# tgialoimtr/cnn_lstm_ctc_ocr

Measured on AMD Instinct MI355X. Metric: line-crops/sec (train step) at 32x256 bs=256; CER vs ref, higher is better.
Workload: dtype bf16

## Files before the change

cnn_lstm_ctc_ocr_amd/csrc/gemm_w4.hip:

```cpp
#include "gemm.h"
#include "mfma_util.h"

namespace ocrk {

namespace {

constexpr unsigned W4_OOB = 0x80000000u;

__device__ __forceinline__ void w4_barrier() {
    __builtin_amdgcn_sched_barrier(0);
    asm volatile("" ::: "memory");
    __builtin_amdgcn_s_barrier();
    asm volatile("" ::: "memory");
    __builtin_amdgcn_sched_barrier(0);
}

template <int NR, int NM, int REST>
__device__ __forceinline__ void w4_interleave() {
#pragma unroll
    for (int r = 0; r < NR; ++r) {
        __builtin_amdgcn_sched_group_barrier(0x8, NM, 0);
        __builtin_amdgcn_sched_group_barrier(0x100, 1, 0);
    }
    __builtin_amdgcn_sched_group_barrier(0x8, REST, 0);
}

typedef unsigned short u16x4 __attribute__((ext_vector_type(4)));

__device__ __forceinline__ i32x4_t w4_rsrc(const void* base, int bytes) {
    const uint64_t b = (uint64_t)base;
    return i32x4_t{(int)(unsigned)b, (int)((unsigned)(b >> 32) & 0xffffu), bytes, 0x00020000};
}

__device__ __forceinline__ void w4_dma16(const i32x4_t& r, unsigned lds, unsigned voff, unsigned soff) {
    asm volatile("s_nop 0\n\tbuffer_load_dwordx4 %0, %1, %2 offen lds"
                 :: "v"(voff), "s"(r), "s"(soff), "{m0}"(lds) : "memory");
}

__global__ void __launch_bounds__(256) gemm_w4_kernel(const GemmParams p) {
    constexpr int BM = 256, BN = 256, BK = 64, ROWB = 128;
    constexpr int A_BYTES = BM * ROWB, BUF = (BM + BN) * ROWB;
    constexpr int NU = 8;
    constexpr int BIAS_OFF = 2 * BUF, STG_OFF = BIAS_OFF + 4 * 1024;
    constexpr int PITCH = 128 * 2 + 16, STG = 16 * PITCH;
    constexpr int NST = 8 * 4;
    extern __shared__ __attribute__((aligned(16))) char smem[];

    const int tid = threadIdx.x, lane = tid & 63;
    const int wave = __builtin_amdgcn_readfirstlane(tid >> 6);
    const int wm = wave >> 1, wn = wave & 1;
    const int i16 = lane & 15, g = lane >> 4, sw = lane & 7;

    const int tm = (p.M + BM - 1) / BM, tn = (p.N + BN - 1) / BN;
    const int nitems = tm * tn * p.batch;
    const int per = (nitems + 7) >> 3;
    const int xcd = blockIdx.x & 7, slot = blockIdx.x >> 3, sp = gridDim.x >> 3;
    const int wend = min(nitems, (xcd + 1) * per);
    int w_issue = xcd * per + slot;
    if (w_issue >= wend) return;

    typedef const __attribute__((address_space(4))) GemmParams* KArgs;
    const bool has_bias = p.bias != nullptr;
    const int c_nk = max(1, (p.K + BK - 1) / BK);

    const int lrow = lane >> 3;
    const int cs = (lane & 7) ^ lrow;
    i32x4_t ra, rb;
    int i_m0 = 0, i_n0 = 0, i_zb = 0, i_kt = 0, i_cnt = 0;
    const unsigned a_lane = (unsigned)(lrow * p.lda * 2), b_lane = (unsigned)(lrow * p.ldb * 2);
    auto setup_issue = [&](int w) {
        const PPItem it = pp_item(w, tm, tn, 1, BM, BN);
        ra = w4_rsrc(reinterpret_cast<const bf16*>(p.A) + it.zb * p.strideA, p.M * (int)p.lda * 2);
        rb = w4_rsrc(reinterpret_cast<const bf16*>(p.B) + it.zb * p.strideB, p.N * (int)p.ldb * 2);
        i_m0 = it.m0;
        i_n0 = it.n0;
        i_zb = it.zb;
        i_kt = 0;
    };
    int ops = 0;
    const unsigned lds0 = (unsigned)(uintptr_t)(__attribute__((address_space(3))) char*)smem;
    auto lane_off = [&](unsigned lane_row, bool on) -> unsigned {
        const int k = i_kt * BK + 8 * cs;
        return on && k < p.K ? lane_row + (unsigned)(k * 2) : W4_OOB;
    };
    auto unit_base = [&](int first, unsigned buf, int& row, unsigned& lds) {
        row = first + wave * 8;
        lds = buf + wave * 8 * ROWB;
        asm volatile("" : "+s"(row), "+s"(lds));
    };
    auto dma_a = [&](int i, int row, unsigned lds, unsigned va) {
        const int mrow = row + i * 32;
        const unsigned soff = mrow < p.M ? (unsigned)(mrow * (int)p.lda * 2) : 0u;
        w4_dma16(ra, lds + i * 32 * ROWB, lrow < p.M - mrow ? va : W4_OOB, soff);
    };
    auto dma_b = [&](int i, int row, unsigned lds, unsigned vb) {
        const int ncol = row + i * 32;
        const unsigned soff = ncol < p.N ? (unsigned)(ncol * (int)p.ldb * 2) : 0u;
        w4_dma16(rb, lds + i * 32 * ROWB, lrow < p.N - ncol ? vb : W4_OOB, soff);
    };
    auto dma_bias = [&](bool on) {
        if (i_kt == 0 && has_bias && wave == 0) {
            const int n = i_n0 + 4 * lane;
            KArgs e = (KArgs)__builtin_amdgcn_kernarg_segment_ptr();
            asm volatile("" : "+s"(e));
            const i32x4_t rbias = w4_rsrc(e->bias + i_zb * e->strideBias, p.N * 4);
            w4_dma16(rbias, lds0 + BIAS_OFF + (i_cnt & 3) * 1024, on && n < p.N ? (unsigned)(n * 4) : W4_OOB, 0u);
            ops += 1;
        }
    };
    auto advance_issue = [&]() -> bool {
        if (++i_kt < c_nk) return true;
        w_issue += sp;
        ++i_cnt;
        if (w_issue >= wend) return false;
        setup_issue(w_issue);
        return true;
    };

    int w_comp = w_issue, c_cnt = 0;

    bf16x8 af0[8], bf0[8], af1[8], bf1[8];
    const int a_base = (wm * 128 + i16) * ROWB, b_base = A_BYTES + (wn * 128 + i16) * ROWB;
    auto read_a = [&](const char* buf, int kk, bf16x8 (&fr)[8]) {
#pragma unroll
        for (int i = 0; i < 8; ++i)
            fr[i] = *reinterpret_cast<const bf16x8*>(buf + a_base + i * 16 * ROWB + (((kk * 4 + g) ^ sw) << 4));
    };
    auto read_b = [&](const char* buf, int kk, bf16x8 (&fr)[8]) {
#pragma unroll
        for (int j = 0; j < 8; ++j)
            fr[j] = *reinterpret_cast<const bf16x8*>(buf + b_base + j * 16 * ROWB + (((kk * 4 + g) ^ sw) << 4));
    };
    floatx4 acc[8][8];
    auto zero_acc = [&]() {
#pragma unroll
        for (int i = 0; i < 8; ++i)
#pragma unroll
            for (int j = 0; j < 8; ++j) acc[i][j] = floatx4{0.f, 0.f, 0.f, 0.f};
    };
    auto mfma_rows = [&](auto I0_, const bf16x8 (&a)[8], const bf16x8 (&b)[8]) {
        constexpr int I0 = decltype(I0_)::value;
#pragma unroll
        for (int i = I0; i < I0 + 4; ++i)
#pragma unroll
            for (int j = 0; j < 8; ++j)
                acc[i][j] = __builtin_amdgcn_mfma_f32_16x16x32_bf16(b[j], a[i], acc[i][j], 0, 0, 0);
    };
    using R0 = std::integral_constant<int, 0>;
    using R4 = std::integral_constant<int, 4>;
    (void)read_b;

    int mA1 = 0, mB1 = 0, mA2 = 0, mB2 = 0;
    setup_issue(w_issue);
    bool more = true;
    int m0done = 0;
#pragma unroll
    for (int t = 0; t < 2; ++t) {
        const unsigned va = lane_off(a_lane, more), vb = lane_off(b_lane, more);
        int row;
        unsigned lds;
        unit_base(i_m0, lds0 + t * BUF, row, lds);
#pragma unroll
        for (int i = 0; i < NU; ++i) dma_a(i, row, lds, va);
        ops += NU;
        mA1 = ops;
        dma_bias(more);
        unit_base(i_n0, lds0 + t * BUF + A_BYTES, row, lds);
#pragma unroll
        for (int i = 0; i < NU; ++i) dma_b(i, row, lds, vb);
        ops += NU;
        mB1 = ops;
        if (t == 0) m0done = ops;
        if (more) more = advance_issue();
    }
    vm_wait_n(ops - m0done);
    w4_barrier();
    read_a(smem, 0, af0);
    read_b(smem, 0, bf0);

    int s = 0;
    for (;;) {
      zero_acc();
      for (int c_kt = 0; c_kt < c_nk; ++c_kt) {
        char* cur = smem + (s & 1) * BUF;
        const char* nxt = smem + ((s + 1) & 1) * BUF;
        __builtin_amdgcn_sched_barrier(0);
        __builtin_amdgcn_s_setprio(1);
        read_a(cur, 1, af1);
        read_b(cur, 1, bf1);
        mfma_rows(R0{}, af0, bf0);
        mfma_rows(R4{}, af0, bf0);
        w4_interleave<16, 3, 16>();
        __builtin_amdgcn_s_setprio(0);
        __builtin_amdgcn_sched_barrier(0);
        asm volatile("s_waitcnt lgkmcnt(0)" ::: "memory");
        vm_wait_fast<NU>(ops - mA1);
        w4_barrier();
        {
            const unsigned va = lane_off(a_lane, more);
            int row;
            unsigned lds;
            unit_base(i_m0, lds0 + (s & 1) * BUF, row, lds);
            __builtin_amdgcn_s_setprio(1);
#pragma unroll
            for (int q = 0; q < 8; ++q) {
                af0[q] = *reinterpret_cast<const bf16x8*>(nxt + a_base + q * 16 * ROWB + ((g ^ sw) << 4));
#pragma unroll
                for (int j = (q & 1) * 4; j < (q & 1) * 4 + 4; ++j)
                    acc[q >> 1][j] = __builtin_amdgcn_mfma_f32_16x16x32_bf16(bf1[j], af1[q >> 1], acc[q >> 1][j], 0, 0, 0);
                dma_a(q, row, lds, va);
                __builtin_amdgcn_sched_barrier(0);
            }
            __builtin_amdgcn_s_setprio(0);
            ops += NU;
            mA2 = ops;
        }
        vm_wait_fast<NU>(ops - mB1);
        w4_barrier();
        {
            const unsigned vb = lane_off(b_lane, more);
            dma_bias(more);
            int row;
            unsigned lds;
            unit_base(i_n0, lds0 + (s & 1) * BUF + A_BYTES, row, lds);
            __builtin_amdgcn_s_setprio(1);
#pragma unroll
            for (int q = 0; q < 8; ++q) {
                bf0[q] = *reinterpret_cast<const bf16x8*>(nxt + b_base + q * 16 * ROWB + ((g ^ sw) << 4));
#pragma unroll
                for (int j = (q & 1) * 4; j < (q & 1) * 4 + 4; ++j)
                    acc[4 + (q >> 1)][j] =
                        __builtin_amdgcn_mfma_f32_16x16x32_bf16(bf1[j], af1[4 + (q >> 1)], acc[4 + (q >> 1)][j], 0, 0, 0);
                dma_b(q, row, lds, vb);
                __builtin_amdgcn_sched_barrier(0);
            }
            __builtin_amdgcn_s_setprio(0);
            ops += NU;
            mB2 = ops;
        }
        if (more) more = advance_issue();
        mA1 = mA2;
        mB1 = mB2;
        ++s;
      }

        {
            int el;
            asm volatile("v_mbcnt_lo_u32_b32 %0, -1, 0\n\tv_mbcnt_hi_u32_b32 %0, -1, %0" : "=v"(el));
            const PPItem cur_it = pp_item(w_comp, tm, tn, 1, BM, BN);
            KArgs e = (KArgs)__builtin_amdgcn_kernarg_segment_ptr();
            asm volatile("" : "+s"(e));
            const int i16 = el & 15, g = el >> 4;
            const char* bslot = smem + BIAS_OFF + (c_cnt & 3) * 1024 + (wn * 128 + 4 * g) * 4;
            floatx4 bv[8];
#pragma unroll
            for (int j = 0; j < 8; ++j) {
                bv[j] = floatx4{0.f, 0.f, 0.f, 0.f};
                if (has_bias) bv[j] = *reinterpret_cast<const floatx4*>(bslot + j * 64);
            }
            char* stg = smem + STG_OFF + wave * STG;
            bf16* Cb = reinterpret_cast<bf16*>(e->C) + cur_it.zb * e->strideC;
            const __amdgpu_buffer_rsrc_t rc =
                __builtin_amdgcn_make_buffer_rsrc(Cb, 0, ((p.M - 1) * (int)e->ldc + p.N) * 2, 0x00020000);
            const int c8 = el & 15, r0 = el >> 4;
            const int n = cur_it.n0 + wn * 128 + 8 * c8;
#pragma unroll
            for (int h = 0; h < 8; ++h) {
#pragma unroll
                for (int j = 0; j < 8; ++j) {
                    floatx4 v = acc[h][j] * e->alpha + bv[j];
                    if (e->relu) {
#pragma unroll
                        for (int r = 0; r < 4; ++r) v[r] = fmaxf(v[r], 0.f);
                    }
                    u16x4 o;
#pragma unroll
                    for (int r = 0; r < 4; ++r) o[r] = __builtin_bit_cast(unsigned short, (bf16)v[r]);
                    *reinterpret_cast<u16x4*>(stg + i16 * PITCH + (j * 16 + 4 * g) * 2) = o;
                }
                __builtin_amdgcn_wave_barrier();
#pragma unroll
                for (int q = 0; q < 4; ++q) {
                    const int r = r0 + q * 4;
                    const int m = cur_it.m0 + wm * 128 + h * 16 + r;
                    const u32x4 v = *reinterpret_cast<const u32x4*>(stg + r * PITCH + c8 * 16);
                    const unsigned off = (m < p.M && n < p.N) ? (unsigned)(((int64_t)m * e->ldc + n) * 2) : W4_OOB;
                    __builtin_amdgcn_raw_buffer_store_b128(v, rc, off, 0, 0);
                }
                __builtin_amdgcn_wave_barrier();
            }
            ops += NST;
        }
        w_comp += sp;
        ++c_cnt;
        if (w_comp >= wend) break;
    }
    vm_wait<0>();
}

}

int gemm_w4(const GemmParams& p, int amode, int bmode, int dtype, hipStream_t stream) {
    const int64_t mode = opt(OPT_GEMM_W4);
    if (mode == 0 || dtype != OCRK_BF16 || amode != A_ROWK || bmode != B_NK) return -1;
    if (!p.c_bf16 || p.accumulate || p.splits != 1 || p.mask || p.stats || p.mask_bits || p.relu_bits) return -1;
    if (p.N % 8 != 0 || p.K % 8 != 0 || (int64_t)p.M < 4096 || p.N < 96) return -1;
    if ((int64_t)p.M * p.lda * 2 >= (1ll << 31) || (int64_t)p.N * p.ldb * 2 >= (1ll << 31) ||
        (int64_t)p.M * p.ldc * 2 >= (1ll << 31))
        return -1;
    if (p.ldc % 8 != 0 || p.strideC % 8 != 0 || (uintptr_t)p.C % 16 != 0) return -1;
    if (p.bias && (uintptr_t)p.bias % 16 != 0) return -1;
    if (p.lda % 8 != 0 || p.ldb % 8 != 0) return -1;
    if (mode == 1 && (p.K < 2048 || p.N < 512)) return -1;
    constexpr int LDS = 2 * 512 * 128 + 4 * 1024 + 4 * 16 * (128 * 2 + 16);
    static DeviceOnce configured;
    set_dyn_lds(configured, reinterpret_cast<const void*>(&gemm_w4_kernel), LDS);
    const int ncu = cu_count();
    const int64_t items = cdiv(p.M, 256) * cdiv(p.N, 256) * (int64_t)p.batch;
    const int64_t grid = std::min<int64_t>(cdiv(items, 8) * 8, (int64_t)(ncu / 8) * 8);
    gemm_w4_kernel<<<dim3((unsigned)grid), 256, LDS, stream>>>(p);
    opt_add(OPT_GEMM_W4_LAUNCHES, 1);
    return launch_status("gemm_w4");
}

}
```

cnn_lstm_ctc_ocr_amd/csrc/gemm_w4tn.hip:

```cpp
#include "gemm.h"
#include "mfma_util.h"

namespace ocrk {

namespace {

constexpr unsigned W4T_OOB = 0x80000000u;

__device__ __forceinline__ void w4t_barrier() {
    __builtin_amdgcn_sched_barrier(0);
    asm volatile("" ::: "memory");
    __builtin_amdgcn_s_barrier();
    asm volatile("" ::: "memory");
    __builtin_amdgcn_sched_barrier(0);
}

__device__ __forceinline__ void w4t_dma16(const i32x4_t& r, unsigned lds, unsigned voff, unsigned soff) {
    asm volatile("s_nop 0\n\tbuffer_load_dwordx4 %0, %1, %2 offen lds"
                 :: "v"(voff), "s"(r), "s"(soff), "{m0}"(lds) : "memory");
}

__global__ void __launch_bounds__(256) gemm_w4tn_kernel(const GemmParams p) {
    constexpr int BM = 256, BN = 256, BK = 64, ROWB = 128, BLK = BK * ROWB;
    constexpr int A_BYTES = 4 * BLK, BUF = 8 * BLK;
    constexpr int NU = 8;
    extern __shared__ __attribute__((aligned(16))) char smem[];

    const int tid = threadIdx.x, lane = tid & 63;
    const int wave = __builtin_amdgcn_readfirstlane(tid >> 6);
    const int wm = wave >> 1, wn = wave & 1;
    const int i16 = lane & 15, g = lane >> 4;

    const int tm = (p.M + BM - 1) / BM, tn = (p.N + BN - 1) / BN;
    const int nT = tm * tn;
    const int nitems = nT * p.batch * p.splits;
    const int per = (nitems + 7) >> 3;
    const int w = (int)(blockIdx.x & 7) * per + (int)(blockIdx.x >> 3);
    if (w >= nitems || (int)(blockIdx.x >> 3) >= per) return;
    const int z = w / nT, t = w - z * nT;
    constexpr int GM = 4;
    const int gsz = GM * tn, grp = t / gsz, first = grp * GM;
    const int gm = min(GM, tm - first), rr = t - grp * gsz;
    const int m0 = (first + rr % gm) * BM, n0 = (rr / gm) * BN;
    const int zb = z / p.splits, zs = z - zb * p.splits;
    const int kbeg = zs * p.k_chunk;
    const int kend = min(p.K, kbeg + p.k_chunk);
    const int nk = max(1, (kend - kbeg + BK - 1) / BK);
    const uint64_t pa = (uint64_t)(reinterpret_cast<const bf16*>(p.A) + zb * p.strideA);
    const uint64_t pb = (uint64_t)(reinterpret_cast<const bf16*>(p.B) + zb * p.strideB);
    const i32x4_t ra = {(int)(unsigned)pa, (int)((unsigned)(pa >> 32) & 0xffffu), p.K * (int)p.lda * 2, 0x00020000};
    const i32x4_t rb = {(int)(unsigned)pb, (int)((unsigned)(pb >> 32) & 0xffffu), p.K * (int)p.ldb * 2, 0x00020000};

    const int lrow = lane >> 3;
    const int chunk = (lane & 7) ^ lrow;
    const unsigned lds0 = (unsigned)(uintptr_t)(__attribute__((address_space(3))) char*)smem;
    unsigned va[2], vb[2];
    int krow[2];
#pragma unroll
    for (int h = 0; h < 2; ++h) {
        krow[h] = (h * 4 + wave) * 8 + lrow;
        va[h] = (unsigned)((krow[h] * (int)p.lda + m0 + 8 * chunk) * 2);
        vb[h] = (unsigned)((krow[h] * (int)p.ldb + n0 + 8 * chunk) * 2);
    }
    auto dma_a = [&](int i, int kt, unsigned buf, bool on) {
        const int k0 = kbeg + kt * BK;
        const bool ok = on && k0 + krow[i & 1] < kend && m0 + 64 * (i >> 1) + 8 * chunk < p.M;
        const unsigned soff = on ? (unsigned)(k0 * (int)p.lda * 2 + 128 * (i >> 1)) : 0u;
        w4t_dma16(ra, buf + (i >> 1) * BLK + ((i & 1) * 4 + wave) * 1024, ok ? va[i & 1] : W4T_OOB, soff);
    };
    auto dma_b = [&](int i, int kt, unsigned buf, bool on) {
        const int k0 = kbeg + kt * BK;
        const bool ok = on && k0 + krow[i & 1] < kend && n0 + 64 * (i >> 1) + 8 * chunk < p.N;
        const unsigned soff = on ? (unsigned)(k0 * (int)p.ldb * 2 + 128 * (i >> 1)) : 0u;
        w4t_dma16(rb, buf + A_BYTES + (i >> 1) * BLK + ((i & 1) * 4 + wave) * 1024, ok ? vb[i & 1] : W4T_OOB, soff);
    };

    const int kr0 = 4 * g + (i16 >> 2), cq = 4 * (i16 & 3);
    auto tr_off = [&](int blk, int col, int kk) {
        const int r = kk * 32 + kr0;
        return blk * BLK + r * ROWB + ((((col >> 3) ^ (r & 7))) << 4) + (col & 7) * 2;
    };
    auto frag_a = [&](const char* buf, int i, int kk) {
        return frag_tr(reinterpret_cast<const unsigned short*>(buf + tr_off(2 * wm + (i >> 2), (i & 3) * 16 + cq, kk)),
                       16 * (ROWB / 2));
    };
    auto frag_b = [&](const char* buf, int j, int kk) {
        return frag_tr(reinterpret_cast<const unsigned short*>(
                           buf + A_BYTES + tr_off(2 * wn + (j >> 2), (j & 3) * 16 + cq, kk)),
                       16 * (ROWB / 2));
    };

    floatx4 acc[8][8];
#pragma unroll
    for (int i = 0; i < 8; ++i)
#pragma unroll
        for (int j = 0; j < 8; ++j) acc[i][j] = floatx4{0.f, 0.f, 0.f, 0.f};
    bf16x8 af0[8], bf0[8], af1[8], bf1[8];

#pragma unroll
    for (int t2 = 0; t2 < 2; ++t2) {
#pragma unroll
        for (int i = 0; i < NU; ++i) dma_a(i, t2, lds0 + t2 * BUF, t2 < nk);
#pragma unroll
        for (int i = 0; i < NU; ++i) dma_b(i, t2, lds0 + t2 * BUF, t2 < nk);
    }
    vm_wait<2 * NU>();
    w4t_barrier();
#pragma unroll
    for (int i = 0; i < 8; ++i) af0[i] = frag_a(smem, i, 0);
#pragma unroll
    for (int j = 0; j < 8; ++j) bf0[j] = frag_b(smem, j, 0);

    for (int kt = 0; kt < nk; ++kt) {
        const char* cur = smem + (kt & 1) * BUF;
        const char* nxt = smem + ((kt + 1) & 1) * BUF;
        const unsigned curl = lds0 + (kt & 1) * BUF;
        const bool more = kt + 2 < nk;
        __builtin_amdgcn_sched_barrier(0);
        __builtin_amdgcn_s_setprio(1);
#pragma unroll
        for (int i = 0; i < 8; ++i) af1[i] = frag_a(cur, i, 1);
#pragma unroll
        for (int j = 0; j < 8; ++j) bf1[j] = frag_b(cur, j, 1);
#pragma unroll
        for (int i = 0; i < 8; ++i)
#pragma unroll
            for (int j = 0; j < 8; ++j)
                acc[i][j] = __builtin_amdgcn_mfma_f32_16x16x32_bf16(bf0[j], af0[i], acc[i][j], 0, 0, 0);
#pragma unroll
        for (int r = 0; r < 24; ++r) {
            __builtin_amdgcn_sched_group_barrier(0x8, 2, 0);
            __builtin_amdgcn_sched_group_barrier(0x100, 1, 0);
        }
#pragma unroll
        for (int r = 0; r < 8; ++r) {
            __builtin_amdgcn_sched_group_barrier(0x8, 1, 0);
            __builtin_amdgcn_sched_group_barrier(0x100, 1, 0);
        }
        __builtin_amdgcn_sched_group_barrier(0x8, 8, 0);
        __builtin_amdgcn_s_setprio(0);
        __builtin_amdgcn_sched_barrier(0);
        asm volatile("s_waitcnt lgkmcnt(0)" ::: "memory");
        vm_wait<NU>();
        w4t_barrier();
        __builtin_amdgcn_s_setprio(1);
#pragma unroll
        for (int q = 0; q < 8; ++q) {
            af0[q] = frag_a(nxt, q, 0);
#pragma unroll
            for (int j = (q & 1) * 4; j < (q & 1) * 4 + 4; ++j)
                acc[q >> 1][j] = __builtin_amdgcn_mfma_f32_16x16x32_bf16(bf1[j], af1[q >> 1], acc[q >> 1][j], 0, 0, 0);
            dma_a(q, kt + 2, curl, more);
            __builtin_amdgcn_sched_barrier(0);
        }
        __builtin_amdgcn_s_setprio(0);
        vm_wait<NU>();
        w4t_barrier();
        __builtin_amdgcn_s_setprio(1);
#pragma unroll
        for (int q = 0; q < 8; ++q) {
            bf0[q] = frag_b(nxt, q, 0);
#pragma unroll
            for (int j = (q & 1) * 4; j < (q & 1) * 4 + 4; ++j)
                acc[4 + (q >> 1)][j] =
                    __builtin_amdgcn_mfma_f32_16x16x32_bf16(bf1[j], af1[4 + (q >> 1)], acc[4 + (q >> 1)][j], 0, 0, 0);
            dma_b(q, kt + 2, curl, more);
            __builtin_amdgcn_sched_barrier(0);
        }
        __builtin_amdgcn_s_setprio(0);
        __builtin_amdgcn_sched_barrier(0);
    }
    vm_wait<0>();

    const int mrow0 = m0 + wm * 128 + i16, ncol0 = n0 + wn * 128 + 4 * g;
    float* C;
    int64_t ldc;
    bool acc_c;
    if (p.splits > 1) {
        C = p.splitk_ws + ((int64_t)zb * p.splits + zs) * (int64_t)p.M * p.N;
        ldc = p.N;
        acc_c = false;
    } else {
        C = reinterpret_cast<float*>(p.C) + zb * p.strideC;
        ldc = p.ldc;
        acc_c = p.accumulate != 0;
    }
#pragma unroll
    for (int i = 0; i < 8; ++i) {
        const int m = mrow0 + i * 16;
        if (m >= p.M) continue;
#pragma unroll
        for (int j = 0; j < 8; ++j) {
            const int n = ncol0 + j * 16;
            if (n >= p.N) continue;
            floatx4* dst = reinterpret_cast<floatx4*>(C + (int64_t)m * ldc + n);
            floatx4 v = acc[i][j] * p.alpha;
            if (acc_c) v += *dst;
            *dst = v;
        }
    }
}

}

int gemm_w4tn(const GemmParams& p, int amode, int bmode, int dtype, hipStream_t stream) {
    const int64_t mode = opt(OPT_GEMM_W4);
    if (mode == 0 || dtype != OCRK_BF16 || amode != A_COLK || bmode != B_KN) return -1;
    if (!gemm_pptn_covers(amode, p.M, p.N, p.convC)) return -1;
    if (p.c_bf16 || p.bias || p.relu || p.mask || p.stats) return -1;
    if (p.ldb % 8 != 0 || p.lda % 8 != 0) return -1;
    if (p.splits == 1 && (p.ldc % 4 != 0 || (uintptr_t)p.C % 16 != 0 || p.strideC % 4 != 0)) return -1;
    if (p.splits > 1 && (uintptr_t)p.splitk_ws % 16 != 0) return -1;
    if ((int64_t)p.K * p.lda * 2 >= (1ll << 31) || (int64_t)p.K * p.ldb * 2 >= (1ll << 31)) return -1;
    constexpr int LDS = 2 * 8 * 64 * 128;
    static DeviceOnce configured;
    set_dyn_lds(configured, reinterpret_cast<const void*>(&gemm_w4tn_kernel), LDS);
    const int64_t items = cdiv(p.M, 256) * cdiv(p.N, 256) * (int64_t)p.batch * p.splits;
    gemm_w4tn_kernel<<<dim3((unsigned)(cdiv(items, 8) * 8)), 256, LDS, stream>>>(p);
    opt_add(OPT_GEMM_W4_LAUNCHES, 1);
    return launch_status("gemm_w4tn");
}

}
```

Before: 54720.

## Add narrow BN=128 w4 GEMM variant and implicit im2col path for w4tn

Templates the w4 GEMM kernel on BN and selects a 128-wide N tile when the 256x256 tile count would leave most CUs idle, to raise occupancy across the device for small problems. Separately, the transposed w4tn kernel gains an implicit im2col A-operand mode that computes 3x3 tap offsets and padding masks on the fly. This lets conv weight-gradient GEMMs skip materialising the im2col buffer. It adds template instantiations and per-tile pixel-tracking arithmetic, and a risk of indexing errors in the new mask logic.

```diff
diff --git a/cnn_lstm_ctc_ocr_amd/csrc/gemm_w4.hip b/cnn_lstm_ctc_ocr_amd/csrc/gemm_w4.hip
--- a/cnn_lstm_ctc_ocr_amd/csrc/gemm_w4.hip
+++ b/cnn_lstm_ctc_ocr_amd/csrc/gemm_w4.hip
@@ -37,13 +37,17 @@
                  :: "v"(voff), "s"(r), "s"(soff), "{m0}"(lds) : "memory");
 }
 
+template <int BN>
 __global__ void __launch_bounds__(256) gemm_w4_kernel(const GemmParams p) {
-    constexpr int BM = 256, BN = 256, BK = 64, ROWB = 128;
+    constexpr int BM = 256, BK = 64, ROWB = 128;
+    constexpr int WN = BN / 2, NJ = WN / 16;
     constexpr int A_BYTES = BM * ROWB, BUF = (BM + BN) * ROWB;
-    constexpr int NU = 8;
-    constexpr int BIAS_OFF = 2 * BUF, STG_OFF = BIAS_OFF + 4 * 1024;
-    constexpr int PITCH = 128 * 2 + 16, STG = 16 * PITCH;
-    constexpr int NST = 8 * 4;
+    constexpr int NU = 8, NUB = BN / 32;
+    constexpr int NB = 2;
+    constexpr int BIAS_OFF = NB * BUF, STG_OFF = BIAS_OFF + 4 * 1024;
+    constexpr int PITCH = WN * 2 + 16, STG = 16 * PITCH;
+    constexpr int CL = WN / 8, RPS = 64 / CL;
+    constexpr int NST = 8 * (16 / RPS);
     extern __shared__ __attribute__((aligned(16))) char smem[];
 
     const int tid = threadIdx.x, lane = tid & 63;
@@ -104,7 +108,7 @@
             KArgs e = (KArgs)__builtin_amdgcn_kernarg_segment_ptr();
             asm volatile("" : "+s"(e));
             const i32x4_t rbias = w4_rsrc(e->bias + i_zb * e->strideBias, p.N * 4);
-            w4_dma16(rbias, lds0 + BIAS_OFF + (i_cnt & 3) * 1024, on && n < p.N ? (unsigned)(n * 4) : W4_OOB, 0u);
+            w4_dma16(rbias, lds0 + BIAS_OFF + (i_cnt & 3) * 1024, on && 4 * lane < BN && n < p.N ? (unsigned)(n * 4) : W4_OOB, 0u);
             ops += 1;
         }
     };
@@ -119,43 +123,42 @@
 
     int w_comp = w_issue, c_cnt = 0;
 
-    bf16x8 af0[8], bf0[8], af1[8], bf1[8];
-    const int a_base = (wm * 128 + i16) * ROWB, b_base = A_BYTES + (wn * 128 + i16) * ROWB;
+    bf16x8 af0[8], bf0[NJ], af1[8], bf1[NJ];
+    const int a_base = (wm * 128 + i16) * ROWB, b_base = A_BYTES + (wn * WN + i16) * ROWB;
     auto read_a = [&](const char* buf, int kk, bf16x8 (&fr)[8]) {
 #pragma unroll
         for (int i = 0; i < 8; ++i)
             fr[i] = *reinterpret_cast<const bf16x8*>(buf + a_base + i * 16 * ROWB + (((kk * 4 + g) ^ sw) << 4));
     };
-    auto read_b = [&](const char* buf, int kk, bf16x8 (&fr)[8]) {
-#pragma unroll
-        for (int j = 0; j < 8; ++j)
+    auto read_b = [&](const char* buf, int kk, bf16x8 (&fr)[NJ]) {
+#pragma unroll
+        for (int j = 0; j < NJ; ++j)
             fr[j] = *reinterpret_cast<const bf16x8*>(buf + b_base + j * 16 * ROWB + (((kk * 4 + g) ^ sw) << 4));
     };
-    floatx4 acc[8][8];
+    floatx4 acc[8][NJ];
     auto zero_acc = [&]() {
 #pragma unroll
         for (int i = 0; i < 8; ++i)
 #pragma unroll
-            for (int j = 0; j < 8; ++j) acc[i][j] = floatx4{0.f, 0.f, 0.f, 0.f};
-    };
-    auto mfma_rows = [&](auto I0_, const bf16x8 (&a)[8], const bf16x8 (&b)[8]) {
+            for (int j = 0; j < NJ; ++j) acc[i][j] = floatx4{0.f, 0.f, 0.f, 0.f};
+    };
+    auto mfma_rows = [&](auto I0_, const bf16x8 (&a)[8], const bf16x8 (&b)[NJ]) {
         constexpr int I0 = decltype(I0_)::value;
 #pragma unroll
         for (int i = I0; i < I0 + 4; ++i)
 #pragma unroll
-            for (int j = 0; j < 8; ++j)
+            for (int j = 0; j < NJ; ++j)
                 acc[i][j] = __builtin_amdgcn_mfma_f32_16x16x32_bf16(b[j], a[i], acc[i][j], 0, 0, 0);
     };
     using R0 = std::integral_constant<int, 0>;
     using R4 = std::integral_constant<int, 4>;
     (void)read_b;
 
-    int mA1 = 0, mB1 = 0, mA2 = 0, mB2 = 0;
+    int mA[NB + 1] = {}, mB[NB + 1] = {};
     setup_issue(w_issue);
     bool more = true;
-    int m0done = 0;
-#pragma unroll
-    for (int t = 0; t < 2; ++t) {
+#pragma unroll
+    for (int t = 0; t < NB; ++t) {
         const unsigned va = lane_off(a_lane, more), vb = lane_off(b_lane, more);
         int row;
         unsigned lds;
@@ -163,17 +166,16 @@
 #pragma unroll
         for (int i = 0; i < NU; ++i) dma_a(i, row, lds, va);
         ops += NU;
-        mA1 = ops;
+        mA[t] = ops;
         dma_bias(more);
         unit_base(i_n0, lds0 + t * BUF + A_BYTES, row, lds);
 #pragma unroll
-        for (int i = 0; i < NU; ++i) dma_b(i, row, lds, vb);
-        ops += NU;
-        mB1 = ops;
-        if (t == 0) m0done = ops;
+        for (int i = 0; i < NUB; ++i) dma_b(i, row, lds, vb);
+        ops += NUB;
+        mB[t] = ops;
         if (more) more = advance_issue();
     }
-    vm_wait_n(ops - m0done);
+    vm_wait_n(ops - mB[0]);
     w4_barrier();
     read_a(smem, 0, af0);
     read_b(smem, 0, bf0);
@@ -190,11 +192,12 @@
         read_b(cur, 1, bf1);
         mfma_rows(R0{}, af0, bf0);
         mfma_rows(R4{}, af0, bf0);
-        w4_interleave<16, 3, 16>();
+        if constexpr (NJ == 8) w4_interleave<16, 3, 16>();
+        else w4_interleave<12, 2, 8>();
         __builtin_amdgcn_s_setprio(0);
         __builtin_amdgcn_sched_barrier(0);
         asm volatile("s_waitcnt lgkmcnt(0)" ::: "memory");
-        vm_wait_fast<NU>(ops - mA1);
+        vm_wait_fast<NUB>(ops - mA[1]);
         w4_barrier();
         {
             const unsigned va = lane_off(a_lane, more);
@@ -206,16 +209,17 @@
             for (int q = 0; q < 8; ++q) {
                 af0[q] = *reinterpret_cast<const bf16x8*>(nxt + a_base + q * 16 * ROWB + ((g ^ sw) << 4));
 #pragma unroll
-                for (int j = (q & 1) * 4; j < (q & 1) * 4 + 4; ++j)
-                    acc[q >> 1][j] = __builtin_amdgcn_mfma_f32_16x16x32_bf16(bf1[j], af1[q >> 1], acc[q >> 1][j], 0, 0, 0);
+                for (int t = q * (NJ / 2); t < (q + 1) * (NJ / 2); ++t)
+                    acc[t / NJ][t % NJ] =
+                        __builtin_amdgcn_mfma_f32_16x16x32_bf16(bf1[t % NJ], af1[t / NJ], acc[t / NJ][t % NJ], 0, 0, 0);
                 dma_a(q, row, lds, va);
                 __builtin_amdgcn_sched_barrier(0);
             }
             __builtin_amdgcn_s_setprio(0);
             ops += NU;
-            mA2 = ops;
+            mA[NB] = ops;
         }
-        vm_wait_fast<NU>(ops - mB1);
+        vm_wait_fast<NU>(ops - mB[1]);
         w4_barrier();
         {
             const unsigned vb = lane_off(b_lane, more);
@@ -225,22 +229,22 @@
             unit_base(i_n0, lds0 + (s & 1) * BUF + A_BYTES, row, lds);
             __builtin_amdgcn_s_setprio(1);
 #pragma unroll
-            for (int q = 0; q < 8; ++q) {
+            for (int q = 0; q < NJ; ++q) {
                 bf0[q] = *reinterpret_cast<const bf16x8*>(nxt + b_base + q * 16 * ROWB + ((g ^ sw) << 4));
 #pragma unroll
-                for (int j = (q & 1) * 4; j < (q & 1) * 4 + 4; ++j)
-                    acc[4 + (q >> 1)][j] =
-                        __builtin_amdgcn_mfma_f32_16x16x32_bf16(bf1[j], af1[4 + (q >> 1)], acc[4 + (q >> 1)][j], 0, 0, 0);
+                for (int t = q * 4; t < q * 4 + 4; ++t)
+                    acc[4 + t / NJ][t % NJ] = __builtin_amdgcn_mfma_f32_16x16x32_bf16(bf1[t % NJ], af1[4 + t / NJ],
+                                                                                      acc[4 + t / NJ][t % NJ], 0, 0, 0);
                 dma_b(q, row, lds, vb);
                 __builtin_amdgcn_sched_barrier(0);
             }
             __builtin_amdgcn_s_setprio(0);
-            ops += NU;
-            mB2 = ops;
+            ops += NUB;
+            mB[NB] = ops;
         }
         if (more) more = advance_issue();
-        mA1 = mA2;
-        mB1 = mB2;
+        mA[1] = mA[2];
+        mB[1] = mB[2];
         ++s;
       }
 
@@ -251,10 +255,10 @@
             KArgs e = (KArgs)__builtin_amdgcn_kernarg_segment_ptr();
             asm volatile("" : "+s"(e));
             const int i16 = el & 15, g = el >> 4;
-            const char* bslot = smem + BIAS_OFF + (c_cnt & 3) * 1024 + (wn * 128 + 4 * g) * 4;
-            floatx4 bv[8];
-#pragma unroll
-            for (int j = 0; j < 8; ++j) {
+            const char* bslot = smem + BIAS_OFF + (c_cnt & 3) * 1024 + (wn * WN + 4 * g) * 4;
+            floatx4 bv[NJ];
+#pragma unroll
+            for (int j = 0; j < NJ; ++j) {
                 bv[j] = floatx4{0.f, 0.f, 0.f, 0.f};
                 if (has_bias) bv[j] = *reinterpret_cast<const floatx4*>(bslot + j * 64);
             }
@@ -262,12 +266,12 @@
             bf16* Cb = reinterpret_cast<bf16*>(e->C) + cur_it.zb * e->strideC;
             const __amdgpu_buffer_rsrc_t rc =
                 __builtin_amdgcn_make_buffer_rsrc(Cb, 0, ((p.M - 1) * (int)e->ldc + p.N) * 2, 0x00020000);
-            const int c8 = el & 15, r0 = el >> 4;
-            const int n = cur_it.n0 + wn * 128 + 8 * c8;
+            const int c8 = el & (CL - 1), r0 = el / CL;
+            const int n = cur_it.n0 + wn * WN + 8 * c8;
 #pragma unroll
             for (int h = 0; h < 8; ++h) {
 #pragma unroll
-                for (int j = 0; j < 8; ++j) {
+                for (int j = 0; j < NJ; ++j) {
                     floatx4 v = acc[h][j] * e->alpha + bv[j];
                     if (e->relu) {
 #pragma unroll
@@ -280,8 +284,8 @@
                 }
                 __builtin_amdgcn_wave_barrier();
 #pragma unroll
-                for (int q = 0; q < 4; ++q) {
-                    const int r = r0 + q * 4;
+                for (int q = 0; q < 16 / RPS; ++q) {
+                    const int r = r0 + q * RPS;
                     const int m = cur_it.m0 + wm * 128 + h * 16 + r;
                     const u32x4 v = *reinterpret_cast<const u32x4*>(stg + r * PITCH + c8 * 16);
                     const unsigned off = (m < p.M && n < p.N) ? (unsigned)(((int64_t)m * e->ldc + n) * 2) : W4_OOB;
@@ -312,13 +316,18 @@
     if (p.bias && (uintptr_t)p.bias % 16 != 0) return -1;
     if (p.lda % 8 != 0 || p.ldb % 8 != 0) return -1;
     if (mode == 1 && (p.K < 2048 || p.N < 512)) return -1;
-    constexpr int LDS = 2 * 512 * 128 + 4 * 1024 + 4 * 16 * (128 * 2 + 16);
-    static DeviceOnce configured;
-    set_dyn_lds(configured, reinterpret_cast<const void*>(&gemm_w4_kernel), LDS);
     const int ncu = cu_count();
-    const int64_t items = cdiv(p.M, 256) * cdiv(p.N, 256) * (int64_t)p.batch;
+    const bool narrow = 2 * cdiv(p.M, 256) * cdiv(p.N, 256) * (int64_t)p.batch <= ncu;
+    const int bn = narrow ? 128 : 256;
+    const int lds = 2 * (256 + bn) * 128 + 4 * 1024 + 4 * 16 * (bn + 16);
+    static DeviceOnce configured[2];
+    const void* kern = narrow ? reinterpret_cast<const void*>(&gemm_w4_kernel<128>)
+                              : reinterpret_cast<const void*>(&gemm_w4_kernel<256>);
+    set_dyn_lds(configured[narrow ? 1 : 0], kern, lds);
+    const int64_t items = cdiv(p.M, 256) * cdiv(p.N, bn) * (int64_t)p.batch;
     const int64_t grid = std::min<int64_t>(cdiv(items, 8) * 8, (int64_t)(ncu / 8) * 8);
-    gemm_w4_kernel<<<dim3((unsigned)grid), 256, LDS, stream>>>(p);
+    if (narrow) gemm_w4_kernel<128><<<dim3((unsigned)grid), 256, lds, stream>>>(p);
+    else gemm_w4_kernel<256><<<dim3((unsigned)grid), 256, lds, stream>>>(p);
     opt_add(OPT_GEMM_W4_LAUNCHES, 1);
     return launch_status("gemm_w4");
 }
diff --git a/cnn_lstm_ctc_ocr_amd/csrc/gemm_w4tn.hip b/cnn_lstm_ctc_ocr_amd/csrc/gemm_w4tn.hip
--- a/cnn_lstm_ctc_ocr_amd/csrc/gemm_w4tn.hip
+++ b/cnn_lstm_ctc_ocr_amd/csrc/gemm_w4tn.hip
@@ -20,7 +20,9 @@
                  :: "v"(voff), "s"(r), "s"(soff), "{m0}"(lds) : "memory");
 }
 
+template <int AM>
 __global__ void __launch_bounds__(256) gemm_w4tn_kernel(const GemmParams p) {
+    constexpr bool IM = AM == A_IM2COL_T;
     constexpr int BM = 256, BN = 256, BK = 64, ROWB = 128, BLK = BK * ROWB;
     constexpr int A_BYTES = 4 * BLK, BUF = 8 * BLK;
     constexpr int NU = 8;
@@ -48,7 +50,8 @@
     const int nk = max(1, (kend - kbeg + BK - 1) / BK);
     const uint64_t pa = (uint64_t)(reinterpret_cast<const bf16*>(p.A) + zb * p.strideA);
     const uint64_t pb = (uint64_t)(reinterpret_cast<const bf16*>(p.B) + zb * p.strideB);
-    const i32x4_t ra = {(int)(unsigned)pa, (int)((unsigned)(pa >> 32) & 0xffffu), p.K * (int)p.lda * 2, 0x00020000};
+    const i32x4_t ra = {(int)(unsigned)pa, (int)((unsigned)(pa >> 32) & 0xffffu),
+                        p.K * (IM ? p.convC : (int)p.lda) * 2, 0x00020000};
     const i32x4_t rb = {(int)(unsigned)pb, (int)((unsigned)(pb >> 32) & 0xffffu), p.K * (int)p.ldb * 2, 0x00020000};
 
     const int lrow = lane >> 3;
@@ -59,11 +62,58 @@
 #pragma unroll
     for (int h = 0; h < 2; ++h) {
         krow[h] = (h * 4 + wave) * 8 + lrow;
-        va[h] = (unsigned)((krow[h] * (int)p.lda + m0 + 8 * chunk) * 2);
+        va[h] = IM ? (unsigned)((krow[h] * p.convC + 8 * chunk) * 2)
+                   : (unsigned)((krow[h] * (int)p.lda + m0 + 8 * chunk) * 2);
         vb[h] = (unsigned)((krow[h] * (int)p.ldb + n0 + 8 * chunk) * 2);
     }
+    unsigned t_bit[4] = {0, 0, 0, 0}, t_sh[4] = {0, 0, 0, 0};
+    int pw[2] = {0, 0}, ph[2] = {0, 0};
+    unsigned pmask[2] = {0, 0};
+    int step_w = 0, step_h = 0;
+    auto tap_mask = [&](int h) {
+        const unsigned cb = 2u | (pw[h] > 0 ? 1u : 0u) | (pw[h] < p.convW - 1 ? 4u : 0u);
+        pmask[h] = (cb << 3) | (ph[h] > 0 ? cb : 0u) | (ph[h] < p.convH - 1 ? cb << 6 : 0u);
+    };
+    if constexpr (IM) {
+#pragma unroll
+        for (int b = 0; b < 4; ++b) {
+            const int col = min(m0 + 64 * b, p.M - 1);
+            const int tap = col / p.convC;
+            t_bit[b] = m0 + 64 * b < p.M ? 1u << tap : 0u;
+            t_sh[b] = (unsigned)((((tap / 3 - 1) * p.convW + tap % 3 - 1) * p.convC + col - tap * p.convC) * 2);
+        }
+#pragma unroll
+        for (int h = 0; h < 2; ++h) {
+            const int k = kbeg + krow[h];
+            pw[h] = k % p.convW;
+            ph[h] = (k / p.convW) % p.convH;
+            tap_mask(h);
+        }
+        step_w = BK % p.convW;
+        step_h = (BK / p.convW) % p.convH;
+    }
+    auto next_pixels = [&]() {
+        if constexpr (IM) {
+#pragma unroll
+            for (int h = 0; h < 2; ++h) {
+                pw[h] += step_w;
+                const bool wrap = pw[h] >= p.convW;
+                pw[h] -= wrap ? p.convW : 0;
+                ph[h] += step_h + (wrap ? 1 : 0);
+                ph[h] -= ph[h] >= p.convH ? p.convH : 0;
+                tap_mask(h);
+            }
+        }
+    };
     auto dma_a = [&](int i, int kt, unsigned buf, bool on) {
         const int k0 = kbeg + kt * BK;
+        if constexpr (IM) {
+            const int b = i >> 1, h = i & 1;
+            const bool ok = on && k0 + krow[h] < kend && (pmask[h] & t_bit[b]) != 0;
+            const unsigned base = (unsigned)(k0 * p.convC * 2) + t_sh[b];
+            w4t_dma16(ra, buf + b * BLK + (h * 4 + wave) * 1024, ok ? va[h] + base : W4T_OOB, 0u);
+            return;
+        }
         const bool ok = on && k0 + krow[i & 1] < kend && m0 + 64 * (i >> 1) + 8 * chunk < p.M;
         const unsigned soff = on ? (unsigned)(k0 * (int)p.lda * 2 + 128 * (i >> 1)) : 0u;
         w4t_dma16(ra, buf + (i >> 1) * BLK + ((i & 1) * 4 + wave) * 1024, ok ? va[i & 1] : W4T_OOB, soff);
@@ -101,6 +151,7 @@
     for (int t2 = 0; t2 < 2; ++t2) {
 #pragma unroll
         for (int i = 0; i < NU; ++i) dma_a(i, t2, lds0 + t2 * BUF, t2 < nk);
+        next_pixels();
 #pragma unroll
         for (int i = 0; i < NU; ++i) dma_b(i, t2, lds0 + t2 * BUF, t2 < nk);
     }
@@ -153,6 +204,7 @@
             dma_a(q, kt + 2, curl, more);
             __builtin_amdgcn_sched_barrier(0);
         }
+        next_pixels();
         __builtin_amdgcn_s_setprio(0);
         vm_wait<NU>();
         w4t_barrier();
@@ -205,18 +257,25 @@
 
 int gemm_w4tn(const GemmParams& p, int amode, int bmode, int dtype, hipStream_t stream) {
     const int64_t mode = opt(OPT_GEMM_W4);
-    if (mode == 0 || dtype != OCRK_BF16 || amode != A_COLK || bmode != B_KN) return -1;
+    const bool im = amode == A_IM2COL_T;
+    if (mode == 0 || dtype != OCRK_BF16 || (amode != A_COLK && !im) || bmode != B_KN) return -1;
     if (!gemm_pptn_covers(amode, p.M, p.N, p.convC)) return -1;
     if (p.c_bf16 || p.bias || p.relu || p.mask || p.stats) return -1;
-    if (p.ldb % 8 != 0 || p.lda % 8 != 0) return -1;
+    if (p.ldb % 8 != 0 || (!im && p.lda % 8 != 0)) return -1;
     if (p.splits == 1 && (p.ldc % 4 != 0 || (uintptr_t)p.C % 16 != 0 || p.strideC % 4 != 0)) return -1;
     if (p.splits > 1 && (uintptr_t)p.splitk_ws % 16 != 0) return -1;
-    if ((int64_t)p.K * p.lda * 2 >= (1ll << 31) || (int64_t)p.K * p.ldb * 2 >= (1ll << 31)) return -1;
+    const int64_t a_bytes = im ? ((int64_t)p.K + 128) * p.convC * 2 : (int64_t)p.K * p.lda * 2;
+    if (a_bytes >= (1ll << 31) || (int64_t)p.K * p.ldb * 2 >= (1ll << 31)) return -1;
+    if (im && (p.batch != 1 || p.convH < 1 || p.convW < 1 || p.M != 9 * p.convC)) return -1;
     constexpr int LDS = 2 * 8 * 64 * 128;
-    static DeviceOnce configured;
-    set_dyn_lds(configured, reinterpret_cast<const void*>(&gemm_w4tn_kernel), LDS);
+    static DeviceOnce configured[2];
+    const void* kern = im ? reinterpret_cast<const void*>(&gemm_w4tn_kernel<A_IM2COL_T>)
+                          : reinterpret_cast<const void*>(&gemm_w4tn_kernel<A_COLK>);
+    set_dyn_lds(configured[im ? 1 : 0], kern, LDS);
     const int64_t items = cdiv(p.M, 256) * cdiv(p.N, 256) * (int64_t)p.batch * p.splits;
-    gemm_w4tn_kernel<<<dim3((unsigned)(cdiv(items, 8) * 8)), 256, LDS, stream>>>(p);
+    const dim3 grid((unsigned)(cdiv(items, 8) * 8));
+    if (im) gemm_w4tn_kernel<A_IM2COL_T><<<grid, 256, LDS, stream>>>(p);
+    else gemm_w4tn_kernel<A_COLK><<<grid, 256, LDS, stream>>>(p);
     opt_add(OPT_GEMM_W4_LAUNCHES, 1);
     return launch_status("gemm_w4tn");
 }
```

Result: faster. 55410, median of 6 (+1.3%).
